# eigenkernel/eigenkernel

Measured on AMD Instinct MI355X. Metric: eigenpairs/s (full spectrum) + achieved fp64 TFLOP/s vs roofline, N=16384 GEP, higher is better.
Workload: dtype f64

## Files before the change

eigenkernel_amd/csrc/ek_common.h:

```cpp
#pragma once
#include <hip/hip_runtime.h>
#include <cstddef>
#include <cstdint>
#include <cstdio>

#define EK_HIP_CHECK(expr)                                                              \
  do {                                                                                  \
    hipError_t _e = (expr);                                                             \
    if (_e != hipSuccess) {                                                             \
      fprintf(stderr, "[ek_hip] %s failed at %s:%d: %s\n", #expr, __FILE__, __LINE__,   \
              hipGetErrorString(_e));                                                   \
      return -1000 - (int)_e;                                                           \
    }                                                                                   \
  } while (0)

namespace ek {

constexpr int kWave = 64;

inline int ceil_div(int a, int b) { return (a + b - 1) / b; }
inline int round_up(int a, int b) { return ceil_div(a, b) * b; }

struct GemmDesc {
  int M, N, K;
// ... 114 lines not shown

constexpr int kMaxTeam = 16;
struct SytrdMember {
  double *A; int lda;
  double *d, *e, *tau;
  double *V; int ldv;
  void *work;
  int rank;
};
struct SytrdExchange {
  int nranks;
  void (*allreduce)(hipStream_t s, int nmem, double *const *bufs, size_t count, void *user);
  void *user;
  void (*allgatherv)(hipStream_t s, int nmem, int rank0, double *const *bufs, const size_t *offs,
                     const size_t *counts, int nranks, void *user) = nullptr;
};
size_t sytrd_dist_work_bytes(int n, int nranks);
void sytrd_lower_dist(hipStream_t s, int n, int nmem, const SytrdMember *mem, const SytrdExchange &x);
void sytrd_team_allreduce(hipStream_t s, int nmem, double *const *bufs, size_t count, void *user);
void team_allgatherv(hipStream_t s, int nmem, int rank0, double *const *bufs, const size_t *offs,
                     const size_t *counts, int nranks, void *user);

void sytrd_debug_split(void *alt, int mask);
void sytrd_set_max_cols(int max_cols);
int sytrd_get_max_cols();
void symv_profile_enable(int stride);
void symv_profile_collect(double *seconds, long long *launches, double *bytes);

constexpr int kBandW = 64;
size_t sy2sb_work_bytes(int n);
void sy2sb_lower(hipStream_t s, hipStream_t s2, int n, double *A, int lda, double *Vall, int ldv, double *tau1,
                 int *d_flag, void *work);
void sy2sb_set_flow(int pair_min, int lookahead_min);

struct Sy2sbMember { double *A; int lda; double *Vall; int ldv; double *tau1; int *d_flag; void *work; int rank; };
size_t sy2sb_dist_work_bytes(int n, int nranks);
void sy2sb_lower_dist(hipStream_t s, hipStream_t s2, int n, int nmem, const Sy2sbMember *mem, const SytrdExchange &x);
void sy2sb_dist_set_lookahead(int min_rows);
void sy2sb_dist_profile(bool on);
void sy2sb_dist_profile_collect(double *seconds, int P);

size_t sb2st_work_bytes(int n, bool with_records = true);
size_t sb2st_record_bytes(int n);
constexpr int kBandLd = 2 * kBandW;
double *sb2st_band(void *work, int n);
void pack_band(hipStream_t s, int n, const double *A, int lda, double *AB );
void sb2st_lower(hipStream_t s, int n, const double *A, int lda, double *d, double *e, double *V2, int ldv2,
                 int *d_flag, void *work, bool band_packed = false, int chase_mode = 0);
void sb2st_apply_q2(hipStream_t s, int n, int ncols, const double *V2, int ldv2, double *Z, int ldz, int *d_flag,
                    void *work, double *records = nullptr);
void sb2st_debug_view(int n, void *work, const double **tau2, int *ldt, const unsigned **ctl);

size_t stedc_work_bytes(int n, int nsel = -1);
bool stedc_compact(int n, int nsel);
int stedc_merge_plan(int n, int nsel, int *tri, int cap, size_t offs[3]);
struct StedcSelect { int nsel, nb, npcol, mycol; int first = 0; };
struct StedcTeam { int nranks; int rank; const SytrdExchange *x; int levels; };
int stedc_team_levels(int n, int nranks);
void stedc_team_set_levels(int levels);
void stedc_team_profile(bool on);
void stedc_team_profile_collect(double *seconds);
void stedc(hipStream_t s, int n, const double *d, const double *e, double *w, double *Z,
           int ldz, void *work, int *d_info, const StedcSelect *sel = nullptr, double *d_flops = nullptr,
           double *wscratch = nullptr, const StedcTeam *team = nullptr);

size_t stebz_work_bytes(int n);
// ... 40 lines not shown
```

eigenkernel_amd/csrc/ek_debug.hip:

```cpp
#include "ek_api_internal.h"

using namespace ek;
using namespace ek::api;

extern "C" {

int ek_hip_potrf_team(int n, double *B_loc, const int desc_B[9], int nteam, long long *mismatch) {
  if (n < 0) return -1;
  if (!B_loc && n > 0) return -2;
  int rc = check_desc(desc_B, 3, n, n); if (rc) return rc;
  if (nteam < 0 || nteam > kMaxTeam) return -4;
  rc = ensure_init(); if (rc) return rc;
  if (mismatch) *mismatch = 0;
  if (n == 0) return 0;
  std::lock_guard<std::mutex> lk(g_mu);
  if (nteam == 0 && !g_comm.on) return -4;
  hipStream_t s = g_ctx.stream;
  const int ld = pad_ld(n), nblk = ceil_div(n, kDiagNB);
  const int nmem = nteam > 0 ? nteam : 1, P = nteam > 0 ? nteam : g_comm.nranks;
  const size_t wb = potrf_dist_work_bytes(n, ld, P);
  const size_t per = al((size_t)ld * ld * 8) + al((size_t)nblk * kDiagNB * kDiagNB * 8) + al(wb) + 256;
  void *ws;
  rc = workspace(per * nmem + 256, &ws);
  if (rc) return rc;
// ... 188 lines not shown
  if (poison && wb >= 8)
    hipLaunchKernelGGL(fill_words_kernel, dim3(256), dim3(256), 0, s, (unsigned long long *)work, wb / 8, 0x7FF8DEADBEEF1234ull);
  sy2sb_lower(s, g_ctx.stream2, n, dA, ld, dV, ld, dt, g_ctx.d_info + 2, work);
  EK_HIP_CHECK(hipGetLastError());
  rc = d2h_matrix(n, n, dA, ld, A, lda, s); if (rc) return rc;
  rc = d2h_matrix(n, n, dV, ld, V, ldv, s); if (rc) return rc;
  if (tau) EK_HIP_CHECK(hipMemcpyAsync(tau, dt, (size_t)n * 8, hipMemcpyDeviceToHost, s));
  int f = 0;
  EK_HIP_CHECK(hipMemcpyAsync(&f, g_ctx.d_info + 2, sizeof(int), hipMemcpyDeviceToHost, s));
  EK_HIP_CHECK(hipStreamSynchronize(s));
  if (flag) *flag = f;
  return 0;
}

int ek_hip_debug_sy2sb(int n, double *A, int lda, double *V, int ldv, double *tau, int *flag) {
  if (n < 1) return -1;
  if (!A || lda < n) return -3;
  if (!V || ldv < n) return -5;
  return sy2sb_on_host_arrays(n, A, lda, V, ldv, tau, 0, flag);
}

int ek_hip_debug_sy2sb_stage(int n, double *A, int lda, double *V, int ldv, double *tau, int poison, int *flag) {
  if (n < 1) return -1;
  if (!A) return -2;
  if (lda < n) return -3;
  if (!V) return -4;
  if (ldv < n) return -5;
  if (!tau) return -6;
  if (!flag) return -8;
  return sy2sb_on_host_arrays(n, A, lda, V, ldv, tau, poison, flag);
}

int ek_hip_debug_set_sy2sb_flow(int pair_min, int lookahead_min) { sy2sb_set_flow(pair_min, lookahead_min); return 0; }

__global__ void band_to_matrix_kernel(int n, const double *__restrict__ AB, double *__restrict__ A, int lda) {
  const int c = blockIdx.x;
  for (int d = threadIdx.x; d <= kBandW; d += blockDim.x)
    if (c + d < n) A[(size_t)(c + d) + (size_t)c * lda] = AB[(size_t)d + (size_t)c * kBandLd];
}

int ek_hip_debug_sy2sb_team(int n, double *A, int lda, double *V, int ldv, double *tau, int nteam, int *flag,
                            long long *mismatch) {
  if (n < 1 || !A || !V || !tau || lda < n || ldv < n) return -1;
  if (nteam < 0 || nteam > kMaxTeam) return -7;
  int rc = ensure_init(); if (rc) return rc;
  std::lock_guard<std::mutex> lk(g_mu);
  if (nteam == 0 && !g_comm.on) return -7;
  hipStream_t s = g_ctx.stream;
  const int ld = pad_ld(n);
  const int nmem = nteam > 0 ? nteam : 1, P = nteam > 0 ? nteam : g_comm.nranks;
  const size_t wb = sy2sb_dist_work_bytes(n, P), bandb = (size_t)kBandLd * (round_up(n + 1, 128)) * 8;
  const size_t per = 2 * al((size_t)ld * ld * 8) + al(wb) + al(bandb) + al((size_t)ld * 8) + 256;
  void *ws;
  rc = workspace(per * nmem + 512, &ws);
  if (rc) return rc;
  Arena a(ws, g_ctx.ws_bytes);
  unsigned long long *d_cnt = a.get<unsigned long long>(1);
  int *d_flags = a.get<int>(kMaxTeam);
  EK_HIP_CHECK(hipMemsetAsync(d_cnt, 0, 8, s));
  EK_HIP_CHECK(hipMemsetAsync(d_flags, 0, kMaxTeam * sizeof(int), s));
  Sy2sbMember mem[kMaxTeam];
  double *ABs[kMaxTeam];
  for (int m = 0; m < nmem; ++m) {
    double *dA = a.get<double>((size_t)ld * ld), *dV = a.get<double>((size_t)ld * ld);
    char *work = a.get<char>(wb);
    ABs[m] = (double *)a.get<char>(bandb);
// ... 687 lines not shown
```

eigenkernel_amd/csrc/ek_sy2sb.hip:

```cpp
#include "ek_common.h"
#include "ek_block64.h"
#include "ek_switch.h"

#include <chrono>
#include <climits>
#include <cstdlib>
#include <vector>

namespace ek {
namespace {

using namespace b64;
static_assert(SB == kBandW, "the panel width is the width of the 64x64 building blocks");
constexpr int CH = 64;
#ifndef EK_CHOLQR_MAXDEV
#define EK_CHOLQR_MAXDEV 0.25
#endif

__device__ __forceinline__ void wave_sync() {
  __builtin_amdgcn_s_waitcnt(0xc07f);
  __builtin_amdgcn_wave_barrier();
}

struct PanelArgs {
  int m;
  const double *src; int lds_;
  const double *M;
  double *dst; int ldd;
  double *Gpart;
  const double *L1;
  const double *Rband;
  double *Vall; int ldv;
  double *Apanel; int lda;
  double *Vd1, *Vd2; int ldi;
  const int *pflag;
  const double *tau;
  double *Tout;
  unsigned *arrived;
  int *nz;
// ... 593 lines not shown
#pragma unroll
      for (int q = 0; q < HB * HB; ++q) x[q] = s_X[q];
      for (int r = jb + t; r < m; r += HT) {
        double v[HB];
#pragma unroll
        for (int k = 0; k < HB; ++k) v[k] = vget(r, jb + k);
#pragma unroll
        for (int c = 0; c < HB; ++c) {
          double acc = 0.0;
#pragma unroll
          for (int k = 0; k < HB; ++k) acc += v[k] * x[k * HB + c];
          P[(size_t)r + (size_t)(c0 + c) * ldp] -= acc;
        }
      }
      __syncthreads();
    }
  }
}

struct SymmArgs {
  int m; const double *A; int lda;
  const double *V; int ldv;
  double *Ypart; int ldy; long long sY;
  int T, tiles_per_split;
  int P, rank, r0;
  int SD = 0, ST = 0;
};
__host__ __device__ inline int symm_dist_chunk(int count, int parts) { return (count + parts - 1) / parts; }
constexpr int BK = 32, MC_LD = 128 + 16, KC_LD = BK + 2;
constexpr int A_TILE = (BK * MC_LD > 128 * KC_LD) ? BK * MC_LD : 128 * KC_LD;
constexpr int V_LD = BK + 2;
typedef double double2_t __attribute__((ext_vector_type(2)));

template <bool DIST>
__global__ __launch_bounds__(256, 2) void symm_lower_kernel(SymmArgs p) {
  __shared__ __attribute__((aligned(16))) double sA[A_TILE];
  __shared__ __attribute__((aligned(16))) double sV[SB * V_LD];
  const int t = threadIdx.x, lane = t & 63, wave = t >> 6, l15 = lane & 15, l4 = lane >> 4;
  int rb = blockIdx.x, ks = blockIdx.y;
  if (DIST) {
    const int b = blockIdx.x, nd = p.T * p.SD;
    if (b < nd) { rb = b / p.SD; ks = b % p.SD; }
    else {
      const int h = (b - nd) / p.ST, j = (b - nd) % p.ST, q = p.r0 >> 7;
      ks = p.SD + j;
      if (p.P == 1) rb = h;
      else {
        const int first = q + ((p.rank - q) % p.P + p.P) % p.P;
        if ((p.r0 & 127) == 0) rb = first + h * p.P - q;
        else rb = first + (h >> 1) * p.P - q - 1 + (h & 1);
      }
      if (rb < 0 || rb >= p.T) return;
    }
  }
  int kt0 = ks * p.tiles_per_split;
  int kt1 = kt0 + p.tiles_per_split; if (kt1 > p.T) kt1 = p.T;
  const int m0 = rb * 128;
  if (DIST) {
    const bool heavy = ((((p.r0 + m0) >> 7) % p.P) == p.rank) || ((((p.r0 + m0 + 64) >> 7) % p.P) == p.rank);
    if (ks < p.SD) {
      const int td = symm_dist_chunk(p.T, p.SD);
      kt0 = ks * td; kt1 = kt0 + td; if (kt1 > rb + 1) kt1 = rb + 1;
      if (kt0 > rb) return;
    } else {
      const int cnt = p.T - rb - 1, len = symm_dist_chunk(cnt > 0 ? cnt : 1, p.ST);
      kt0 = rb + 1 + (ks - p.SD) * len; kt1 = kt0 + len; if (kt1 > p.T) kt1 = p.T;
      if (!heavy || kt0 >= kt1) return;
    }
  }
  const int wm = (wave & 1) * 64, wn = (wave >> 1) * 32;
// ... 515 lines not shown
  if (c0 < cs) c0 = cs;
  int M = 0, N = 0;
  if (c0 < n) {
    M = n - (int)c0;
    long long cend = (long long)(S + 1) * 128;
    if (cend > n) cend = n;
    N = (int)(cend - c0);
  }
  const size_t e = (size_t)panel * maxb + k;
  offs[3 * e] = c0 - r0; offs[3 * e + 1] = c0 - r0; offs[3 * e + 2] = c0 * ((long long)lda + 1);
  dims[3 * e] = M; dims[3 * e + 1] = N; dims[3 * e + 2] = 2 * SB;
}

struct DistProf {
  bool on = false;
  std::vector<hipEvent_t> ev;
  std::vector<int> kind;
  hipEvent_t mark(hipStream_t st) {
    hipEvent_t e = nullptr;
    if (hipEventCreate(&e) != hipSuccess) return nullptr;
    (void)hipEventRecord(e, st);
    ev.push_back(e);
    return e;
  }
};
DistProf g_dprof;
int g_dist_la_min = -1;
int g_flow_pair_min = -1, g_flow_la_min = -1;

}

size_t sy2sb_work_bytes(int n) { return Layout(n).total; }
void sy2sb_set_flow(int pair_min, int lookahead_min) { g_flow_pair_min = pair_min; g_flow_la_min = lookahead_min; }

void sy2sb_lower(hipStream_t s, hipStream_t s2, int n, double *A, int lda, double *Vall, int ldv, double *tau1,
                 int *d_flag, void *work) {
  if (n <= 2) return;
  ensure_attrs();
  static bool evs = false;
  static hipEvent_t evA[2], evB[2], evC, evD;
  if (!evs) {
    for (int q = 0; q < 2; ++q) {
      (void)hipEventCreateWithFlags(&evA[q], hipEventDisableTiming);
      (void)hipEventCreateWithFlags(&evB[q], hipEventDisableTiming);
    }
    (void)hipEventCreateWithFlags(&evC, hipEventDisableTiming);
    (void)hipEventCreateWithFlags(&evD, hipEventDisableTiming);
    evs = true;
  }
  const Layout L(n);
  char *w = (char *)work;
  double *opA[2] = {(double *)(w + L.off_opa[0]), (double *)(w + L.off_opa[1])};
  double *opB[2] = {(double *)(w + L.off_opb[0]), (double *)(w + L.off_opb[1])};
  double *Qt = (double *)(w + L.off_qt), *Y = (double *)(w + L.off_y);
  double *Ypart = (double *)(w + L.off_ypart), *Gpart = (double *)(w + L.off_gpart);
  double *Cg1 = (double *)(w + L.off_cg1), *Cg2 = (double *)(w + L.off_cg2);
  double *sm = (double *)(w + L.off_small);
  double *Gred = sm, *R1 = sm + 4096, *R1inv = sm + 2 * 4096, *M2 = sm + 3 * 4096, *L1 = sm + 5 * 4096, *Rband = sm + 6 * 4096;
  double *Tm[2][2] = {{sm + 4 * 4096, sm + 7 * 4096}, {sm + 9 * 4096, sm + 8 * 4096}};
  double *G1 = sm + 14 * 4096, *G2 = sm + 15 * 4096;
  double *Gpart2 = (double *)(w + L.off_gpart2), *Gred2 = sm + 11 * 4096;
  const int ldi = L.mpad;
  constexpr int staged_max = 8192;
  const int la_min = g_flow_la_min < 0 ? switch_int(kSwLookaheadMin) : (g_flow_la_min == 0 ? INT_MAX : g_flow_la_min);
  constexpr int small_max = 4096;
  const int pair_min = g_flow_pair_min < 0 ? switch_int(kSwPairMin) : g_flow_pair_min;
// ... 267 lines not shown
```

eigenkernel_amd/solver.py:

```python
import ctypes
import os
from dataclasses import dataclass, field

import numpy as np

from . import descriptor as _d

_HERE = os.path.dirname(os.path.abspath(__file__))
LIB_PATH = os.environ.get("EK_HIP_LIB") or os.path.join(_HERE, "csrc", "libek_hip.so")

N_STAGES = 8
SOLVERS = ("hip", "hip_select", "general_hip", "general_hip_select")
REPLACES = {"hip": "scalapack", "hip_select": "scalapack_select",
            "general_hip": "general_scalapack", "general_hip_select": "general_scalapack_select"}


class LibraryMissing(RuntimeError):
    pass


_lib = None
_dp = ctypes.POINTER(ctypes.c_double)
_ip = ctypes.POINTER(ctypes.c_int)
_llp = ctypes.POINTER(ctypes.c_longlong)
# ... 46 lines not shown
        "ek_hip_ormtr": (c_int, [c_int, c_int, _dp, _ip, _dp, _dp, _ip]),
        "ek_hip_trtrs": (c_int, [c_int, c_int, _dp, _ip, _dp, _ip]),
        "ek_hip_dgemm": (c_int, [c_int, c_int, c_int, c_int, c_int, c_dbl, _dp, c_int, _dp, c_int,
                                 c_dbl, _dp, c_int, c_int]),
        "ek_hip_malloc": (c_int, [ctypes.POINTER(vp), c_ull]),
        "ek_hip_free": (c_int, [vp]),
        "ek_hip_memcpy_h2d": (c_int, [vp, vp, c_ull]),
        "ek_hip_memcpy_d2h": (c_int, [vp, vp, c_ull]),
        "ek_hip_synchronize": (c_int, []),
        "ek_hip_synth_matrix_device": (c_int, [c_int, c_ull, vp, c_int]),
        "ek_hip_residual_device": (c_int, [c_int, c_int, c_int, vp, c_int, vp, c_int, vp, vp, c_int, _dp, _dp, _dp]),
        "ek_hip_orthogonality_device": (c_int, [c_int, c_int, c_int, c_int, vp, c_int, vp, c_int, _dp]),
        "ek_hip_ipratios_device": (c_int, [c_int, c_int, c_int, vp, c_int, vp, c_int, _dp]),
        "ek_hip_check": (c_int, [c_int, c_int, c_int, c_int, c_int, c_int, _dp, _ip, _dp, _ip, _dp, _dp, _ip, _dp]),
        "ek_hip_profile_symv": (c_int, [c_int]),
        "ek_hip_debug_sytrd": (c_int, [c_int, c_int, c_int, _dp]),
        "ek_hip_debug_sytrd_team": (c_int, [c_int, c_int, c_int, _dp]),
        "ek_hip_debug_set_sytrd_maxcols": (c_int, [c_int]),
        "ek_hip_debug_sytrd_work_bytes": (ctypes.c_ulonglong, [c_int]),
        "ek_hip_debug_sytrd_split": (c_int, [vp, c_int]),
        "ek_hip_debug_gemm_at": (c_int, [c_int, c_int, c_int, c_int, c_int, vp, c_int, vp, c_int, c_dbl, vp, c_int,
                                         c_int, c_int, _dp]),
        "ek_hip_debug_sytrd_at": (c_int, [c_int, c_int, c_int, vp, vp, vp, _dp]),
        "ek_hip_debug_gemm_desc": (c_int, [c_int] * 5 + [c_dbl, c_dbl, vp, c_int, c_ll, vp, c_int, c_ll, vp, c_int, c_ll]
                                   + [c_int] * 5 + [_llp, _ip, _ip]),
        "ek_hip_debug_gemm_plan": (c_int, [c_int] * 5 + [c_dbl, c_dbl, vp, c_int, c_ll, vp, c_int, c_ll, vp, c_int, c_ll]
                                   + [c_int] * 5 + [_llp, _ip, _ip]),
        "ek_hip_debug_gemm_compact_map": (c_int, [c_int, c_int, c_ll, c_int, _ip, _ip, _ip]),
        "ek_hip_debug_reduce_team": (c_int, [c_int, c_int, c_int, _dp]),
        "ek_hip_profile_symv_get": (c_int, [_dp, ctypes.POINTER(ctypes.c_longlong), _dp]),
        "ek_hip_debug_sy2sb": (c_int, [c_int, _dp, c_int, _dp, c_int, _dp, _ip]),
        "ek_hip_debug_sy2sb_stage": (c_int, [c_int, _dp, c_int, _dp, c_int, _dp, c_int, _ip]),
        "ek_hip_debug_set_sy2sb_flow": (c_int, [c_int, c_int]),
        "ek_hip_debug_sb2st": (c_int, [c_int, _dp, c_int, _dp, _dp, _dp, c_int, c_int, _ip]),
        "ek_hip_debug_sb2st_stage": (c_int, [c_int, _dp, c_int, c_int, c_int, _dp, _dp, _dp, c_int, _dp, c_int, _dp, c_int,
                                             c_int, _ip, _ip]),
        "ek_hip_debug_two_stage_timing": (c_int, [c_int, c_int, c_int, _dp, _ip]),
        "ek_hip_debug_set_two_stage": (c_int, [c_int]),
        "ek_hip_profile_kernels": (c_int, [c_int]),
        "ek_hip_profile_kernels_get": (c_int, [_dp, _llp]),
        "ek_hip_debug_last_solve_stats": (c_int, [_dp, c_int]),
        "ek_hip_debug_sy2sb_team": (c_int, [c_int, _dp, c_int, _dp, c_int, _dp, c_int, _ip, _llp]),
        "ek_hip_debug_sy2sb_team_timing": (c_int, [c_int, c_int, c_int, _dp]),
        "ek_hip_debug_sy2sb_team_profile": (c_int, [c_int, c_int, c_int, c_int, _dp, _dp]),
        "ek_hip_debug_fail_next_chase": (c_int, [c_int]),
        "ek_hip_debug_stedc_team": (c_int, [c_int, c_int, c_int]),
        "ek_hip_debug_potrf_team_profile": (c_int, [c_int, c_int]),
        "ek_hip_debug_potrf_team_profile_get": (c_int, [c_int, _dp]),
        "ek_hip_debug_stedc_team_get": (c_int, [_dp]),
        "ek_hip_debug_stedc": (c_int, [c_int, _dp, _dp, c_int, c_int, c_int, c_int, c_int, _dp, _dp, c_int, _ip, c_int,
                                       _ip]),
        "ek_hip_debug_stedc_zcols": (c_int, [c_int, c_int]),
        "ek_hip_debug_ormtr": (c_int, [c_int, c_int, _dp, c_int, _dp, _dp, c_int, c_int, c_int]),
        "ek_hip_debug_last_pipe_stats": (c_int, [_dp, c_int]),
        "ek_hip_debug_workspace_bytes": (ctypes.c_ulonglong, [c_int, c_int, c_int, c_int, ctypes.POINTER(ctypes.c_ulonglong)]),
        "ek_hip_eigenvalues_device": (c_int, [c_int, c_int, c_int, c_int, vp, c_int, vp, c_int, vp, _dp, c_int]),
        "ek_hip_eigenvalues": (c_int, [c_int, c_int, c_int, c_int, _dp, c_int, _dp, c_int, _dp, _dp, c_int]),
        "ek_hip_stebz": (c_int, [c_int, _dp, _dp, c_int, c_int, _dp]),
        "ek_hip_debug_values_workspace_bytes": (ctypes.c_ulonglong, [c_int, c_int]),
        "ek_hip_debug_set_stebz": (c_int, [c_int]),
        "ek_hip_eigenpairs_device": (c_int, [c_int, c_int, c_int, c_int, c_dbl, c_dbl, c_int, c_int, vp, c_int, vp, c_int,
                                             _ip, _ip, vp, vp, c_int, c_int, _dp, c_int]),
        "ek_hip_eigenpairs": (c_int, [c_int, c_int, c_int, c_int, c_dbl, c_dbl, c_int, c_int, _dp, c_int, _dp, c_int,
                                      _ip, _ip, _dp, _dp, c_int, c_int, _dp, c_int]),
        "ek_hip_stebz_range": (c_int, [c_int, _dp, _dp, c_dbl, c_dbl, _ip, _ip, _dp]),
        "ek_hip_debug_window_workspace_bytes": (ctypes.c_ulonglong, [c_int, c_int, c_int, c_int, c_int]),
# ... 107 lines not shown
        "ek_hip_check_sparse": (c_int, [c_int, c_int, c_ll, _ip, _dp, c_ll, _ip, _dp, _dp, _dp, c_int,
                                        c_int, c_int, c_int, c_int, _dp, _dp]),
        "ek_hip_sparse_to_dense": (c_int, [c_int, c_ll, _ip, _dp, _dp, c_int]),
        "ek_hip_debug_sparse_check_workspace_bytes": (c_ull, [c_int, c_int, c_ll, c_ll, c_int, c_int, c_int, c_int]),
        "ek_hip_debug_sparse_csr": (c_ll, [c_int, c_ll, _ip, _dp, _llp, _ip, _dp]),
    }
    for name, (res, args) in sigs.items():
        try:
            fn = getattr(lib, name)
        except AttributeError:
            if os.environ.get("EK_HIP_BRINGUP") == "1":
                continue
            raise
        fn.restype = res
        fn.argtypes = args
    if path is None:
        _lib = lib
    return lib


EXPORTED_SYMBOLS = (
    "ek_hip_version", "ek_hip_init", "ek_hip_finalize", "ek_hip_stage_name", "ek_hip_solve",
    "ek_hip_solve_device", "ek_hip_solve_replicated", "ek_hip_solve_device_grid",
    "ek_hip_set_allgatherv", "ek_hip_gather_matrix", "ek_hip_potrf", "ek_hip_sygst", "ek_hip_sytrd", "ek_hip_stedc",
    "ek_hip_ormtr", "ek_hip_trtrs", "ek_hip_dgemm", "ek_hip_malloc", "ek_hip_free",
    "ek_hip_memcpy_h2d", "ek_hip_memcpy_d2h", "ek_hip_synchronize", "ek_hip_synth_matrix_device",
    "ek_hip_profile_symv", "ek_hip_profile_symv_get", "ek_hip_debug_sytrd",
    "ek_hip_residual_device", "ek_hip_orthogonality_device", "ek_hip_ipratios_device", "ek_hip_check",
    "ek_hip_sytrd_team", "ek_hip_comm_unique_id", "ek_hip_comm_init", "ek_hip_comm_size", "ek_hip_comm_rank",
    "ek_hip_comm_destroy", "ek_hip_comm_allreduce_device", "ek_hip_debug_sytrd_team", "ek_hip_sygst_team",
    "ek_hip_potrf_team", "ek_hip_debug_reduce_team", "ek_hip_comm_attach_host",
    "ek_hip_debug_set_sytrd_maxcols", "ek_hip_debug_sytrd_work_bytes", "ek_hip_debug_sytrd_at", "ek_hip_debug_sytrd_split", "ek_hip_debug_gemm_at",
    "ek_hip_debug_gemm_desc", "ek_hip_debug_gemm_plan", "ek_hip_debug_gemm_compact_map",
    "ek_hip_debug_sy2sb", "ek_hip_debug_sy2sb_stage", "ek_hip_debug_set_sy2sb_flow", "ek_hip_debug_sb2st", "ek_hip_debug_sb2st_stage", "ek_hip_debug_two_stage_timing", "ek_hip_debug_set_two_stage",
    "ek_hip_profile_kernels", "ek_hip_profile_kernels_get", "ek_hip_debug_last_solve_stats",
    "ek_hip_debug_sy2sb_team", "ek_hip_debug_sy2sb_team_timing", "ek_hip_debug_sy2sb_team_profile", "ek_hip_debug_workspace_bytes", "ek_hip_debug_fail_next_chase", "ek_hip_debug_last_pipe_stats",
    "ek_hip_debug_stedc_team", "ek_hip_debug_stedc_team_get", "ek_hip_debug_stedc",
    "ek_hip_debug_stedc_zcols", "ek_hip_debug_ormtr",
    "ek_hip_debug_potrf_team_profile", "ek_hip_debug_potrf_team_profile_get",
    "ek_hip_eigenvalues_device", "ek_hip_eigenvalues", "ek_hip_stebz",
    "ek_hip_debug_values_workspace_bytes", "ek_hip_debug_set_stebz",
    "ek_hip_eigenpairs_device", "ek_hip_eigenpairs", "ek_hip_stebz_range", "ek_hip_debug_window_workspace_bytes",
    "ek_hip_sygvx_device", "ek_hip_sygvx", "ek_hip_sygst_ibtype", "ek_hip_trmm", "ek_hip_debug_sygvx_workspace_bytes",
    "ek_hip_eigenpairs_batched_device", "ek_hip_eigenpairs_batched",
    "ek_hip_eigenpairs_vbatched_device", "ek_hip_eigenpairs_vbatched",
    "ek_hip_debug_vbatched_streams", "ek_hip_debug_vbatched_last",
    "ek_hip_check_batched_device", "ek_hip_check_batched", "ek_hip_check_vbatched_device", "ek_hip_check_vbatched",
    "ek_hip_sygv_batched_device", "ek_hip_sygv_batched", "ek_hip_sygv_vbatched_device", "ek_hip_sygv_vbatched",
    "ek_hip_check_sygv_batched_device", "ek_hip_check_sygv_batched", "ek_hip_check_sygv_vbatched_device",
    "ek_hip_check_sygv_vbatched", "ek_hip_check_sygvx_device", "ek_hip_check_sygvx",
    "ek_hip_eigenpairs_xbatched_device", "ek_hip_eigenpairs_xbatched", "ek_hip_debug_xbatched_chunk",
    "ek_hip_check_xbatched_device", "ek_hip_check_xbatched", "ek_hip_debug_check_xbatched_chunk",
    "ek_hip_sygv_xbatched_device", "ek_hip_sygv_xbatched",
    "ek_hip_check_sygv_xbatched_device", "ek_hip_check_sygv_xbatched",
    "ek_hip_eigenpairs_xvbatched_device", "ek_hip_eigenpairs_xvbatched", "ek_hip_sygv_xvbatched_device",
    "ek_hip_sygv_xvbatched", "ek_hip_debug_xvbatched_last",
    "ek_hip_eigenpairs_window_xvbatched_device", "ek_hip_eigenpairs_window_xvbatched",
    "ek_hip_sygv_window_xvbatched_device", "ek_hip_sygv_window_xvbatched", "ek_hip_debug_window_xvbatched_budget",
    "ek_hip_check_xvbatched_device", "ek_hip_check_xvbatched", "ek_hip_check_sygv_xvbatched_device",
    "ek_hip_check_sygv_xvbatched", "ek_hip_debug_check_xvbatched_last",
    "ek_hip_debug_stage_leaves256", "ek_hip_debug_set_sygst_direct", "ek_hip_debug_sygst_scratch",
    "ek_hip_solve_sparse", "ek_hip_check_sparse_device", "ek_hip_check_sparse", "ek_hip_sparse_to_dense",
    "ek_hip_debug_sparse_check_workspace_bytes", "ek_hip_debug_sparse_csr",
    "ek_hip_eigenpairs_window_batched_device", "ek_hip_eigenpairs_window_batched", "ek_hip_debug_window_batched_chunk",
    "ek_hip_eigenpairs_window_xbatched_device", "ek_hip_eigenpairs_window_xbatched",
    "ek_hip_debug_window_xbatched_chunk",
    "ek_hip_sygv_window_batched_device", "ek_hip_sygv_window_batched",
# ... 898 lines not shown
    ld = max(n, 1)
    info = lib.ek_hip_check_sygvx(int(itype), n, m, _P(A_), ld, _P(B_), ld, _P(wv), _P(Z_), ld, _P(out), _P(q))
    if info:
        raise RuntimeError("ek_hip_check_sygvx info=%d" % info)
    return out, q


def sy2sb(A):
    lib = load_library()
    A = np.array(_farr(A), order="F", copy=True)
    n = A.shape[0]
    V = np.zeros((n, n), order="F"); tau = np.zeros(max(n, 1)); flag = ctypes.c_int(-1)
    rc = lib.ek_hip_debug_sy2sb(n, _P(A), max(1, n), _P(V), max(1, n), _P(tau), ctypes.byref(flag))
    if rc:
        raise RuntimeError("ek_hip_debug_sy2sb info=%d" % rc)
    return A, V, tau[:n], flag.value


def sy2sb_stage(A, poison=False):
    lib = load_library()
    A = np.array(_farr(A), order="F", copy=True)
    n = A.shape[0]
    V = np.zeros((n, n), order="F"); tau = np.zeros(max(n, 1)); flag = ctypes.c_int(-1)
    rc = lib.ek_hip_debug_sy2sb_stage(n, _P(A), max(1, n), _P(V), max(1, n), _P(tau), 1 if poison else 0, ctypes.byref(flag))
    if rc:
        raise RuntimeError("ek_hip_debug_sy2sb_stage info=%d" % rc)
    return A, V, tau[:n], flag.value


def set_sy2sb_flow(pair_min=-1, lookahead_min=-1):
    rc = load_library().ek_hip_debug_set_sy2sb_flow(int(pair_min), int(lookahead_min))
    if rc:
        raise RuntimeError("ek_hip_debug_set_sy2sb_flow info=%d" % rc)


def sy2sb_team(A, nteam):
    lib = load_library()
    A = np.array(_farr(A), order="F", copy=True)
    n = A.shape[0]
    V = np.zeros((n, n), order="F"); tau = np.zeros(max(n, 1)); flag = ctypes.c_int(-1); mism = ctypes.c_longlong(-1)
    rc = lib.ek_hip_debug_sy2sb_team(n, _P(A), max(1, n), _P(V), max(1, n), _P(tau), int(nteam), ctypes.byref(flag),
                                     ctypes.byref(mism))
    if rc:
        raise RuntimeError("ek_hip_debug_sy2sb_team info=%d" % rc)
    return A, V, tau[:n], flag.value, mism.value


def sb2st(Bd, Z=None):
    lib = load_library()
    Bd = np.array(_farr(Bd), order="F", copy=True)
    n = Bd.shape[0]
    d = np.zeros(max(n, 1)); e = np.zeros(max(n, 1)); flag = ctypes.c_int(-1)
    if Z is None:
        rc = lib.ek_hip_debug_sb2st(n, _P(Bd), max(1, n), _P(d), _P(e), None, max(1, n), 0, ctypes.byref(flag))
    else:
        Z = np.array(_farr(Z), order="F", copy=True)
        rc = lib.ek_hip_debug_sb2st(n, _P(Bd), max(1, n), _P(d), _P(e), _P(Z), max(1, n), Z.shape[1], ctypes.byref(flag))
    if rc:
        raise RuntimeError("ek_hip_debug_sb2st info=%d" % rc)
    return d[:n], e[:max(n - 1, 0)], Z, flag.value


def sb2st_stage(Bd, Z=None, form=0, chase_mode=0, reflectors=True, pad=0):
    lib = load_library()
    Bd = _farr(Bd)
    n = Bd.shape[0]
# ... 228 lines not shown
```

include/ek_hip_debug.h:

```cpp
#ifndef EK_HIP_DEBUG_H
#define EK_HIP_DEBUG_H

#ifdef __cplusplus
extern "C" {
#endif

int ek_hip_profile_symv(int enable);
int ek_hip_profile_symv_get(double *seconds, long long *launches, double *algorithmic_bytes);

int ek_hip_profile_kernels(int enable);
int ek_hip_profile_kernels_get(double *seconds , long long *launches );

int ek_hip_debug_sytrd(int n, int ld, int reps, double *seconds);
unsigned long long ek_hip_debug_sytrd_work_bytes(int n);
int ek_hip_debug_sytrd_at(int n, int max_cols, int reps, double *dA, void *work, double *vecs, double *seconds);
int ek_hip_debug_gemm_at(int transa, int transb, int m, int n, int k, const double *dA, int lda, const double *dB,
                         int ldb, double beta, double *dC, int ldc, int lower_only, int reps, double *seconds);
int ek_hip_debug_gemm_desc(int transa, int transb, int m, int n, int k, double alpha, double beta, const double *dA, int lda,
                           long long strideA, const double *dB, int ldb, long long strideB, double *dC, int ldc,
                           long long strideC, int batch, int lower_only, int staged_rank_k, int small_tiles, int even_offs,
                           const long long *offs, const int *dims, int *variant );
int ek_hip_debug_gemm_plan(int transa, int transb, int m, int n, int k, double alpha, double beta, const double *dA, int lda,
                           long long strideA, const double *dB, int ldb, long long strideB, double *dC, int ldc,
                           long long strideC, int batch, int lower_only, int staged_rank_k, int small_tiles, int even_offs,
                           const long long *offs, const int *dims, int *variant );
int ek_hip_debug_gemm_compact_map(int tiles_m, int tiles_n, long long first, int count, int *tm, int *tn, int *valid);
int ek_hip_debug_sytrd_split(void *alt, int mask);
int ek_hip_debug_set_sytrd_maxcols(int max_cols);
int ek_hip_debug_sytrd_team(int n, int nteam, int reps, double *seconds);
int ek_hip_debug_reduce_team(int n, int nteam, int reps, double *seconds );

int ek_hip_debug_sy2sb(int n, double *A, int lda, double *V, int ldv, double *tau, int *flag);
int ek_hip_debug_sb2st(int n, const double *A, int lda, double *d, double *e, double *Z, int ldz, int ncols, int *flag);
int ek_hip_debug_two_stage_timing(int n, int ncols, int reps, double *seconds, int *flag);
int ek_hip_debug_set_two_stage(int min_order);
int ek_hip_debug_sy2sb_stage(int n, double *A, int lda, double *V, int ldv, double *tau, int poison, int *flag);
int ek_hip_debug_set_sy2sb_flow(int pair_min, int lookahead_min);
int ek_hip_debug_sb2st_stage(int n, const double *A, int lda, int form, int chase_mode, double *d, double *e, double *V2,
                             int ldv2, double *tau2, int ldtau, double *Z, int ldz, int ncols, int *ran, int *flag);
int ek_hip_debug_sy2sb_team(int n, double *A, int lda, double *V, int ldv, double *tau, int nteam, int *flag,
                            long long *mismatch);
int ek_hip_debug_sy2sb_team_timing(int n, int nteam, int reps, double *seconds);
int ek_hip_debug_sy2sb_team_profile(int n, int nteam, int reps, int lookahead_min, double *seconds, double *parts);

int ek_hip_debug_last_solve_stats(double *out, int count);

unsigned long long ek_hip_debug_workspace_bytes(int problem, int n, int n_vec, int nranks, unsigned long long *parts);

unsigned long long ek_hip_debug_values_workspace_bytes(int problem, int n);
int ek_hip_debug_set_stebz(int lanes);
unsigned long long ek_hip_debug_window_workspace_bytes(int problem, int n, int jobz, int range, int m);
unsigned long long ek_hip_debug_sygvx_workspace_bytes(int itype, int n, int jobz, int range, int m);
unsigned long long ek_hip_debug_sparse_check_workspace_bytes(int problem, int n, long long nnzA, long long nnzB,
                                                             int n_check, int index1, int index2, int n_ipr);
long long ek_hip_debug_sparse_csr(int n, long long nnz, const int *suf, const double *val, long long *rowptr, int *col,
                                  double *csr_val);
int ek_hip_debug_vbatched_streams(int streams);
int ek_hip_debug_vbatched_last(double *class_seconds, int *class_count);
int ek_hip_debug_xvbatched_last(double *class_seconds, int *class_count);
int ek_hip_debug_xbatched_chunk(int problems);
int ek_hip_debug_window_batched_chunk(int problems);
int ek_hip_debug_window_xbatched_chunk(int problems);
long long ek_hip_debug_window_xvbatched_budget(long long bytes);
int ek_hip_debug_check_xbatched_chunk(int problems);
int ek_hip_debug_check_xvbatched_last(double class_seconds[4], int class_count[4]);

int ek_hip_debug_stage_leaves256(int mode);
int ek_hip_debug_set_sygst_direct(int order);
unsigned long long ek_hip_debug_sygst_scratch(int n, unsigned long long *need );

// ... 22 lines not shown
```

Measured before the change: 20510.

## Rewrite single-device SYMM kernel with register-prefetched interior runs and mixed-layout tiles

```diff
diff --git a/eigenkernel_amd/csrc/ek_common.h b/eigenkernel_amd/csrc/ek_common.h
--- a/eigenkernel_amd/csrc/ek_common.h
+++ b/eigenkernel_amd/csrc/ek_common.h
@@ -170,6 +170,9 @@
 void sy2sb_lower(hipStream_t s, hipStream_t s2, int n, double *A, int lda, double *Vall, int ldv, double *tau1,
                  int *d_flag, void *work);
 void sy2sb_set_flow(int pair_min, int lookahead_min);
+size_t sy2sb_symm_work_bytes(int m);
+void sy2sb_symm(hipStream_t s, int m, const double *A22, int lda, const double *V, int ldv, int tiles_per_split, double *Y,
+                int ldy, void *work);
 
 struct Sy2sbMember { double *A; int lda; double *Vall; int ldv; double *tau1; int *d_flag; void *work; int rank; };
 size_t sy2sb_dist_work_bytes(int n, int nranks);
diff --git a/eigenkernel_amd/csrc/ek_debug.hip b/eigenkernel_amd/csrc/ek_debug.hip
--- a/eigenkernel_amd/csrc/ek_debug.hip
+++ b/eigenkernel_amd/csrc/ek_debug.hip
@@ -244,6 +244,27 @@
 }
 
 int ek_hip_debug_set_sy2sb_flow(int pair_min, int lookahead_min) { sy2sb_set_flow(pair_min, lookahead_min); return 0; }
+
+int ek_hip_debug_symm(int m, const double *dA22, int lda, const double *dV, int ldv, int tiles_per_split, double *dY, int ldy) {
+  if (m < 1) return -1;
+  if (!dA22) return -2;
+  if (lda < m) return -3;
+  if (!dV) return -4;
+  if (ldv < m) return -5;
+  if (tiles_per_split < 1 || (m + 127) / 128 > 16 * (long long)tiles_per_split) return -6;
+  if (!dY) return -7;
+  if (ldy < m) return -8;
+  int rc = ensure_init(); if (rc) return rc;
+  std::lock_guard<std::mutex> lk(g_mu);
+  hipStream_t s = g_ctx.stream;
+  void *ws;
+  rc = workspace(sy2sb_symm_work_bytes(m), &ws);
+  if (rc) return rc;
+  sy2sb_symm(s, m, dA22, lda, dV, ldv, tiles_per_split, dY, ldy, ws);
+  EK_HIP_CHECK(hipGetLastError());
+  EK_HIP_CHECK(hipStreamSynchronize(s));
+  return 0;
+}
 
 __global__ void band_to_matrix_kernel(int n, const double *__restrict__ AB, double *__restrict__ A, int lda) {
   const int c = blockIdx.x;
diff --git a/eigenkernel_amd/csrc/ek_sy2sb.hip b/eigenkernel_amd/csrc/ek_sy2sb.hip
--- a/eigenkernel_amd/csrc/ek_sy2sb.hip
+++ b/eigenkernel_amd/csrc/ek_sy2sb.hip
@@ -5,6 +5,7 @@
 #include <chrono>
 #include <climits>
 #include <cstdlib>
+#include <type_traits>
 #include <vector>
 
 namespace ek {
@@ -664,10 +665,175 @@
 constexpr int V_LD = BK + 2;
 typedef double double2_t __attribute__((ext_vector_type(2)));
 
+enum { kDirect = 0, kTransposed = 1 };
+
+template <bool kc>
+__device__ __forceinline__ void symm_store_slab(double *sA, double *sV, int t, const double2_t (&ra)[8],
+                                                const double2_t (&rv)[4]) {
+#pragma unroll
+  for (int i = 0; i < 8; ++i) {
+    if (kc) { const int k = 2 * (t & 15), x = (t >> 4) + 16 * i; *reinterpret_cast<double2_t *>(&sA[x * KC_LD + k]) = ra[i]; }
+    else    { const int x = 2 * (t & 63), k = (t >> 6) + 4 * i; *reinterpret_cast<double2_t *>(&sA[k * MC_LD + x]) = ra[i]; }
+  }
+#pragma unroll
+  for (int i = 0; i < 4; ++i) { const int k = 2 * (t & 15), nn = (t >> 4) + 16 * i; *reinterpret_cast<double2_t *>(&sV[nn * V_LD + k]) = rv[i]; }
+}
+
+template <bool kc>
+__device__ __forceinline__ void symm_mfma_slab(const double *sA, const double *sV, int wm, int wn, int l15, int l4,
+                                               double4_t (&acc)[2][4]) {
+#pragma unroll
+  for (int kk = 0; kk < BK; kk += 4) {
+    double fa[4], fb[2];
+#pragma unroll
+    for (int i = 0; i < 4; ++i) {
+      const int x = wm + i * 16 + l15, k = kk + l4;
+      fa[i] = kc ? sA[x * KC_LD + k] : sA[k * MC_LD + x];
+    }
+#pragma unroll
+    for (int i = 0; i < 2; ++i) fb[i] = sV[(wn + i * 16 + l15) * V_LD + kk + l4];
+#pragma unroll
+    for (int ni = 0; ni < 2; ++ni)
+#pragma unroll
+      for (int mi = 0; mi < 4; ++mi)
+        acc[ni][mi] = __builtin_amdgcn_mfma_f64_16x16x4f64(fb[ni], fa[mi], acc[ni][mi], 0, 0, 0);
+  }
+}
+
+__device__ __forceinline__ void symm_walk(const SymmArgs &p, double *sA, double *sV) {
+  const int t = threadIdx.x, lane = t & 63, wave = __builtin_amdgcn_readfirstlane(t >> 6), l15 = lane & 15, l4 = lane >> 4;
+  const int rb = blockIdx.x, ks = blockIdx.y;
+  const int kt0 = ks * p.tiles_per_split;
+  int kt1 = kt0 + p.tiles_per_split; if (kt1 > p.T) kt1 = p.T;
+  const int m0 = rb * 128;
+  const int wm = (wave & 1) * 64, wn = (wave >> 1) * 32;
+  double4_t acc[2][4];
+#pragma unroll
+  for (int i = 0; i < 2; ++i)
+#pragma unroll
+    for (int j = 0; j < 4; ++j) acc[i][j] = (double4_t){0.0, 0.0, 0.0, 0.0};
+  double2_t ra[8], rv[4];
+  const bool vec_ok = (((p.lda | p.ldv) & 1) == 0) && ((((size_t)p.A | (size_t)p.V) & 15) == 0);
+  const bool rows_in = vec_ok && m0 + 128 <= p.m;
+  auto fetch_generic = [&](int kt, int k0) {
+    int tq = t;
+    asm volatile("" : "+v"(tq));
+    const int mode = (kt < rb) ? 0 : (kt > rb ? 1 : 2);
+    const int gk0 = kt * 128 + k0;
+    if (mode == 0 && rows_in && gk0 + BK <= p.m) {
+      const double *base = p.A + (size_t)(m0 + 2 * (tq & 63)) + (size_t)(gk0 + (tq >> 6)) * p.lda;
+#pragma unroll
+      for (int i = 0; i < 8; ++i) ra[i] = *reinterpret_cast<const double2_t *>(base + (size_t)(4 * i) * p.lda);
+    } else if (mode == 1 && rows_in && gk0 + BK <= p.m) {
+      const double *base = p.A + (size_t)(gk0 + 2 * (tq & 15)) + (size_t)(m0 + (tq >> 4)) * p.lda;
+#pragma unroll
+      for (int i = 0; i < 8; ++i) ra[i] = *reinterpret_cast<const double2_t *>(base + (size_t)(16 * i) * p.lda);
+    } else {
+#pragma unroll
+      for (int i = 0; i < 8; ++i) {
+        double v[2];
+#pragma unroll
+        for (int h = 0; h < 2; ++h) {
+          int x, k;
+          if (mode == 1) { k = 2 * (tq & 15) + h; x = (tq >> 4) + 16 * i; } else { x = 2 * (tq & 63) + h; k = (tq >> 6) + 4 * i; }
+          const int gx = m0 + x, gk = gk0 + k;
+          double e = 0.0;
+          if (gx < p.m && gk < p.m) {
+            const bool low = (mode == 0) || (mode == 2 && gx >= gk);
+            e = low ? p.A[(size_t)gx + (size_t)gk * p.lda] : p.A[(size_t)gk + (size_t)gx * p.lda];
+          }
+          v[h] = e;
+        }
+        ra[i] = (double2_t){v[0], v[1]};
+      }
+    }
+    if (vec_ok && gk0 + BK <= p.m) {
+      const double *base = p.V + (size_t)(gk0 + 2 * (tq & 15)) + (size_t)(tq >> 4) * p.ldv;
+#pragma unroll
+      for (int i = 0; i < 4; ++i) rv[i] = *reinterpret_cast<const double2_t *>(base + (size_t)(16 * i) * p.ldv);
+    } else {
+#pragma unroll
+      for (int i = 0; i < 4; ++i) {
+        const int gk = gk0 + 2 * (tq & 15), nn = (tq >> 4) + 16 * i;
+        rv[i] = (double2_t){gk < p.m ? p.V[(size_t)gk + (size_t)nn * p.ldv] : 0.0,
+                            gk + 1 < p.m ? p.V[(size_t)gk + 1 + (size_t)nn * p.ldv] : 0.0};
+      }
+    }
+  };
+  auto advance = [&](int &kt, int &k0) -> bool {
+    k0 += BK;
+    if (k0 >= 128 || kt * 128 + k0 >= p.m) { kt += 1; k0 = 0; }
+    return kt < kt1 && kt * 128 < p.m;
+  };
+  auto interior_run = [&](auto kind, int gk0, int n) {
+    constexpr int KIND = decltype(kind)::value;
+    int tq = t;
+    asm volatile("" : "+v"(tq));
+    const char *ua = KIND == kDirect ? (const char *)(p.A + (size_t)m0 + (size_t)(gk0 + BK + wave) * p.lda)
+                                     : (const char *)(p.A + (size_t)(gk0 + BK) + (size_t)(m0 + 4 * wave) * p.lda);
+    const char *uv = (const char *)(p.V + (size_t)(gk0 + BK) + (size_t)(4 * wave) * p.ldv);
+    const unsigned la = KIND == kDirect ? 16u * (unsigned)(tq & 63) : 8u * (unsigned)(2 * (tq & 15) + ((tq >> 4) & 3) * p.lda);
+    const unsigned lv = 8u * (unsigned)(2 * (tq & 15) + ((tq >> 4) & 3) * p.ldv);
+    const size_t sa = (size_t)p.lda * (KIND == kDirect ? 32 : 128), sv = (size_t)p.ldv * 128;
+    const size_t bump = KIND == kDirect ? (size_t)p.lda * (8 * BK) : (size_t)(8 * BK);
+    for (int s = 0; s < n; ++s) {
+      __syncthreads();
+      symm_store_slab<KIND == kTransposed>(sA, sV, t, ra, rv);
+      __syncthreads();
+#pragma unroll
+      for (int i = 0; i < 8; ++i) ra[i] = *reinterpret_cast<const double2_t *>(ua + i * sa + la);
+#pragma unroll
+      for (int i = 0; i < 4; ++i) rv[i] = *reinterpret_cast<const double2_t *>(uv + i * sv + lv);
+      ua += bump; uv += 8 * BK;
+      symm_mfma_slab<KIND == kTransposed>(sA, sV, wm, wn, l15, l4, acc);
+    }
+  };
+  const int dend = (kt1 < rb ? kt1 : rb) * 128, tend = kt1 * 128 < p.m ? kt1 * 128 : p.m;
+  int kt = kt0, k0 = 0;
+  bool fetch = kt0 < kt1, pending = false, pending_kc = false;
+  while (true) {
+    if (fetch) fetch_generic(kt, k0);
+    if (pending) {
+      if (pending_kc) symm_mfma_slab<true>(sA, sV, wm, wn, l15, l4, acc);
+      else symm_mfma_slab<false>(sA, sV, wm, wn, l15, l4, acc);
+    }
+    if (!fetch) break;
+    if (rows_in && kt != rb) {
+      const int gk0 = kt * 128 + k0;
+      const int n = (((kt < rb ? dend : tend) - gk0) >> 5) - 1;
+      if (n > 0) {
+        if (kt > rb) interior_run(std::integral_constant<int, kTransposed>{}, gk0, n);
+        else interior_run(std::integral_constant<int, kDirect>{}, gk0, n);
+        const int g = gk0 + n * BK;
+        kt = g >> 7; k0 = g & 127;
+      }
+    }
+    __syncthreads();
+    if (kt > rb) symm_store_slab<true>(sA, sV, t, ra, rv);
+    else symm_store_slab<false>(sA, sV, t, ra, rv);
+    __syncthreads();
+    pending = true; pending_kc = kt > rb;
+    fetch = advance(kt, k0);
+  }
+  double *Y = p.Ypart + (size_t)ks * p.sY;
+#pragma unroll
+  for (int ni = 0; ni < 2; ++ni)
+#pragma unroll
+    for (int mi = 0; mi < 4; ++mi) {
+      const int mrow = m0 + wm + mi * 16 + l15;
+#pragma unroll
+      for (int r = 0; r < 4; ++r) {
+        const int nn = wn + ni * 16 + l4 + 4 * r;
+        if (mrow < p.m) Y[(size_t)mrow + (size_t)nn * p.ldy] = acc[ni][mi][r];
+      }
+    }
+}
+
 template <bool DIST>
 __global__ __launch_bounds__(256, 2) void symm_lower_kernel(SymmArgs p) {
   __shared__ __attribute__((aligned(16))) double sA[A_TILE];
   __shared__ __attribute__((aligned(16))) double sV[SB * V_LD];
+  if constexpr (!DIST) { symm_walk(p, sA, sV); return; }
   const int t = threadIdx.x, lane = t & 63, wave = t >> 6, l15 = lane & 15, l4 = lane >> 4;
   int rb = blockIdx.x, ks = blockIdx.y;
   if (DIST) {
@@ -1249,6 +1415,21 @@
 
 size_t sy2sb_work_bytes(int n) { return Layout(n).total; }
 void sy2sb_set_flow(int pair_min, int lookahead_min) { g_flow_pair_min = pair_min; g_flow_la_min = lookahead_min; }
+
+size_t sy2sb_symm_work_bytes(int m) {
+  const int mpad = round_up(m > 0 ? m : 1, 128);
+  return al256((size_t)16 * mpad * SB * 8) + al256((size_t)(mpad / CH + 1) * SB * SB * 8);
+}
+void sy2sb_symm(hipStream_t s, int m, const double *A22, int lda, const double *V, int ldv, int tiles_per_split, double *Y,
+                int ldy, void *work) {
+  const int mpad = round_up(m, 128), T = ceil_div(m, 128), nsplit = ceil_div(T, tiles_per_split), nch = ceil_div(m, CH);
+  double *Ypart = (double *)work, *Gpart = (double *)((char *)work + al256((size_t)16 * mpad * SB * 8));
+  SymmArgs sy{m, A22, lda, V, ldv, Ypart, mpad, (long long)mpad * SB, T, tiles_per_split, 1, 0, 0};
+  hipLaunchKernelGGL(symm_lower_kernel<false>, dim3(T, nsplit), dim3(256), 0, s, sy);
+  YredArgs ya{m, nsplit, Ypart, mpad, (long long)mpad * SB, Y, V, ldv, Gpart};
+  ya.ldyo = ldy;
+  hipLaunchKernelGGL(yred_q_kernel, dim3(nch, 4), dim3(256), 0, s, ya);
+}
 
 void sy2sb_lower(hipStream_t s, hipStream_t s2, int n, double *A, int lda, double *Vall, int ldv, double *tau1,
                  int *d_flag, void *work) {
diff --git a/eigenkernel_amd/solver.py b/eigenkernel_amd/solver.py
--- a/eigenkernel_amd/solver.py
+++ b/eigenkernel_amd/solver.py
@@ -102,6 +102,7 @@
         "ek_hip_debug_sy2sb": (c_int, [c_int, _dp, c_int, _dp, c_int, _dp, _ip]),
         "ek_hip_debug_sy2sb_stage": (c_int, [c_int, _dp, c_int, _dp, c_int, _dp, c_int, _ip]),
         "ek_hip_debug_set_sy2sb_flow": (c_int, [c_int, c_int]),
+        "ek_hip_debug_symm": (c_int, [c_int, vp, c_int, vp, c_int, c_int, vp, c_int]),
         "ek_hip_debug_sb2st": (c_int, [c_int, _dp, c_int, _dp, _dp, _dp, c_int, c_int, _ip]),
         "ek_hip_debug_sb2st_stage": (c_int, [c_int, _dp, c_int, c_int, c_int, _dp, _dp, _dp, c_int, _dp, c_int, _dp, c_int,
                                              c_int, _ip, _ip]),
@@ -275,7 +276,7 @@
     "ek_hip_potrf_team", "ek_hip_debug_reduce_team", "ek_hip_comm_attach_host",
     "ek_hip_debug_set_sytrd_maxcols", "ek_hip_debug_sytrd_work_bytes", "ek_hip_debug_sytrd_at", "ek_hip_debug_sytrd_split", "ek_hip_debug_gemm_at",
     "ek_hip_debug_gemm_desc", "ek_hip_debug_gemm_plan", "ek_hip_debug_gemm_compact_map",
-    "ek_hip_debug_sy2sb", "ek_hip_debug_sy2sb_stage", "ek_hip_debug_set_sy2sb_flow", "ek_hip_debug_sb2st", "ek_hip_debug_sb2st_stage", "ek_hip_debug_two_stage_timing", "ek_hip_debug_set_two_stage",
+    "ek_hip_debug_sy2sb", "ek_hip_debug_sy2sb_stage", "ek_hip_debug_set_sy2sb_flow", "ek_hip_debug_symm", "ek_hip_debug_sb2st", "ek_hip_debug_sb2st_stage", "ek_hip_debug_two_stage_timing", "ek_hip_debug_set_two_stage",
     "ek_hip_profile_kernels", "ek_hip_profile_kernels_get", "ek_hip_debug_last_solve_stats",
     "ek_hip_debug_sy2sb_team", "ek_hip_debug_sy2sb_team_timing", "ek_hip_debug_sy2sb_team_profile", "ek_hip_debug_workspace_bytes", "ek_hip_debug_fail_next_chase", "ek_hip_debug_last_pipe_stats",
     "ek_hip_debug_stedc_team", "ek_hip_debug_stedc_team_get", "ek_hip_debug_stedc",
@@ -1240,6 +1241,36 @@
     rc = load_library().ek_hip_debug_set_sy2sb_flow(int(pair_min), int(lookahead_min))
     if rc:
         raise RuntimeError("ek_hip_debug_set_sy2sb_flow info=%d" % rc)
+
+
+def symm_stage(A22, V, tiles_per_split, lda=None, v_shift=0):
+    lib = load_library()
+    A22 = _farr(A22); V = _farr(V)
+    m = A22.shape[0]
+    lda = int(lda) if lda is not None else m + (m & 1)
+    ldv = m + (m & 1)
+    hA = np.full((lda, m), np.nan, order="F"); hA[:m, :] = A22
+    hV = np.full(ldv * 64 + v_shift, np.nan); hV[v_shift:].reshape(64, ldv)[:, :m] = V.T
+    hY = np.full((m, 64), np.nan, order="F")
+    ptrs = []
+
+    def put(a):
+        p = ctypes.c_void_p()
+        if lib.ek_hip_malloc(ctypes.byref(p), a.nbytes) or lib.ek_hip_memcpy_h2d(p, a.ctypes.data, a.nbytes):
+            raise RuntimeError("ek_hip_malloc / ek_hip_memcpy_h2d failed")
+        ptrs.append(p)
+        return p
+    try:
+        dA, dV, dY = put(hA), put(hV), put(hY)
+        rc = lib.ek_hip_debug_symm(m, dA, lda, ctypes.c_void_p(dV.value + 8 * v_shift), ldv, int(tiles_per_split), dY, m)
+        if rc:
+            raise RuntimeError("ek_hip_debug_symm info=%d" % rc)
+        if lib.ek_hip_memcpy_d2h(hY.ctypes.data, dY, hY.nbytes):
+            raise RuntimeError("ek_hip_memcpy_d2h failed")
+    finally:
+        for p in ptrs:
+            lib.ek_hip_free(p)
+    return hY
 
 
 def sy2sb_team(A, nteam):
diff --git a/include/ek_hip_debug.h b/include/ek_hip_debug.h
--- a/include/ek_hip_debug.h
+++ b/include/ek_hip_debug.h
@@ -36,6 +36,7 @@
 int ek_hip_debug_set_two_stage(int min_order);
 int ek_hip_debug_sy2sb_stage(int n, double *A, int lda, double *V, int ldv, double *tau, int poison, int *flag);
 int ek_hip_debug_set_sy2sb_flow(int pair_min, int lookahead_min);
+int ek_hip_debug_symm(int m, const double *dA22, int lda, const double *dV, int ldv, int tiles_per_split, double *dY, int ldy);
 int ek_hip_debug_sb2st_stage(int n, const double *A, int lda, int form, int chase_mode, double *d, double *e, double *V2,
                              int ldv2, double *tau2, int ldtau, double *Z, int ldz, int ncols, int *ran, int *flag);
 int ek_hip_debug_sy2sb_team(int n, double *A, int lda, double *V, int ldv, double *tau, int nteam, int *flag,
```

Result: no change. 20620 (median of 6 runs) (+0.5%).
